# NUS-HPC-AI-Lab/VideoSys

Measured on AMD Instinct MI355X. Metric: videos/min (Open-Sora 512x512x64f, 30 denoise steps, DiT denoising only) + sec/denoise-step, higher is better.
Workload: dtype bf16; 1 GPU; open-sora-v1.2 STDiT3-XL/2 512x512x64f, latent [4,19,64,64], CFG batch 2 = 38912 token rows, 300 text tokens, depth 28; steps_per_video=30, parallelism=dsp1

## Files before the change

videosys_amd/csrc/gemm2_bf16.hip:

```cpp
#include "common.h"
#include "vsys_internal.h"

namespace vsys {
namespace {

constexpr int BM = 256, BK = 32;
constexpr int A_SLOT = BM * BK * 2;
constexpr int W_BASE = 3 * A_SLOT;
constexpr int OUT_ROW_BYTES = 96 * 2 + 16;
constexpr int OUT_WAVE_BYTES = 64 * OUT_ROW_BYTES;

template <int NWN>
struct G2 {
  static constexpr int NW = 2 * NWN;
  static constexpr int NT = 64 * NW;
  static constexpr int BN = 96 * NWN;
  static constexpr int NA = 16 / NW;
  static constexpr int W_SLOT = BN * BK * 2;
  static constexpr int WLEAD = NWN == 4 ? 2 : 1;
  static constexpr int NWSLOT = WLEAD + 1;
  static constexpr int STAGING = W_BASE + NWSLOT * W_SLOT;
  static constexpr int LDS_BYTES = STAGING > NW * OUT_WAVE_BYTES ? STAGING : NW * OUT_WAVE_BYTES;
  static constexpr int LN_BYTES = (BM + BN) * 8;
  static constexpr int KW_BYTES = 160;
};

template <int EPI, int NWN, int STAMP = 0, int MF = 0>
__global__ __launch_bounds__(G2<NWN>::NT, 2) void gemm2_kernel(GemmParams p) {
  using G = G2<NWN>;
  constexpr int BN = G::BN, NA = G::NA, W_SLOT = G::W_SLOT, WLEAD = G::WLEAD;
#if __HIP_DEVICE_COMPILE__
  extern __shared__ __attribute__((aligned(16))) char smem[];
  const int tid = threadIdx.x, lane = tid & 63, wave = tid >> 6;
  const int wm = wave / NWN, wn = wave % NWN;
  const int l31 = lane & 31, hi = lane >> 5;
  const int l15 = lane & 15, lq = lane >> 4;
  static_assert(!MF || (EPI != EPI_F32_SLICES && !STAMP), "the 16x16x32 form covers the token-row epilogues only");
  static_assert(EPI != EPI_LN_QKV_KV || (MF && NWN == 2), "the K/V epilogue exists on the 256 x 192 tile of the 16x16x32 form only");
  const int wave_u = __builtin_amdgcn_readfirstlane(wave);
  const int nbn = p.N / BN;
  int tile = xcd_remap(blockIdx.x, gridDim.x);
  int kslice = 0;
  if constexpr (EPI == EPI_F32_SLICES) {
    const int ntile = ((p.M + BM - 1) / BM) * nbn;
    kslice = tile / ntile;
    tile -= kslice * ntile;
  }
  int bm, bn;
  gemm_raster(tile, (p.M + BM - 1) / BM, nbn, p.raster_gw, p.raster_ph, bm, bn);
  const int row0 = bm * BM, col0 = bn * BN;

  const int dchunk = ((lane & 3) ^ (MF ? ((0x78 >> (2 * ((lane >> 4) & 3))) & 3) : ((lane >> 4) & 3))) * 16;
  int a_off[NA], b_off[3];
#pragma unroll
  for (int i = 0; i < NA; ++i) {
    const int r = wave_u * (16 * NA) + i * 16 + (lane >> 2);
    const int rl = row0 + r < p.M ? r : p.M - 1 - row0;
    a_off[i] = rl * (int)p.lda * 2 + dchunk;
  }
#pragma unroll
  for (int i = 0; i < 3; ++i) b_off[i] = (wave_u * 48 + i * 16 + (lane >> 2)) * (int)p.ldw * 2 + dchunk;
  const int64_t a_bytes = ((int64_t)(p.M - 1 - row0) * p.lda + p.K) * 2, b_bytes = ((int64_t)(p.N - 1 - col0) * p.ldw + p.K) * 2;
  const auto rsrc_a = __builtin_amdgcn_make_buffer_rsrc((void*)(p.A + (int64_t)row0 * p.lda), 0,
                                                        (int)(a_bytes < 0x7fffffff ? a_bytes : 0x7fffffff), 0x00020000);
  const auto rsrc_b = __builtin_amdgcn_make_buffer_rsrc((void*)(p.W + (int64_t)col0 * p.ldw), 0,
                                                        (int)(b_bytes < 0x7fffffff ? b_bytes : 0x7fffffff), 0x00020000);
  typedef __attribute__((address_space(3))) void* lds_ptr_t;
  const int kbase2 = EPI == EPI_F32_SLICES ? kslice * p.ks * 2 : 0;
  auto dma_a = [&](int i, int t, int slot) {
    __builtin_amdgcn_raw_ptr_buffer_load_lds(rsrc_a, (lds_ptr_t)(smem + slot * A_SLOT + (wave_u * (16 * NA) + i * 16) * 64), 16, a_off[i],
                                             kbase2 + t * (BK * 2), 0, 0);
  };
  auto dma_w = [&](int i, int t, int slot) {
    __builtin_amdgcn_raw_ptr_buffer_load_lds(rsrc_b, (lds_ptr_t)(smem + W_BASE + slot * W_SLOT + (wave_u * 48 + i * 16) * 64), 16,
                                             b_off[i], kbase2 + t * (BK * 2), 0, 0);
  };

  const int fsw = MF ? ((lq ^ ((0x78 >> (2 * ((l15 >> 2) & 3))) & 3)) << 4) : ((hi ^ ((l31 >> 2) & 3)) << 4);
  const int frow = MF ? l15 : l31;
  const int xo = (wm * 128 + frow) * 64 + fsw;
  const int wo = W_BASE + (wn * 96 + frow) * 64 + fsw;

  f32x16 acc[MF ? 1 : 4][MF ? 1 : 3];
  f32x4 acc16[MF ? 8 : 1][MF ? 6 : 1];
#pragma unroll
  for (int i = 0; i < (MF ? 1 : 4); ++i)
#pragma unroll
    for (int j = 0; j < (MF ? 1 : 3); ++j)
#pragma unroll
      for (int r = 0; r < 16; ++r) acc[i][j][r] = 0.f;
// ... 181 lines not shown
    }
    __builtin_amdgcn_s_barrier();
    __builtin_amdgcn_sched_barrier(0);
    if constexpr (STAMP) {
      const uint64_t now = __builtin_amdgcn_s_memtime();
      st_bar += now - st_t0; st_t0 = now;
      __builtin_amdgcn_sched_barrier(0);
    }
    sa = sa1;
    sw = sw1;
  }

  if constexpr (EPI == EPI_F32_SLICES) {
    float* o32 = p.out32 + (int64_t)kslice * p.slab;
    const int ncol0 = col0 + wn * 96;
#pragma unroll
    for (int i = 0; i < 4; ++i) {
      const int n = row0 + wm * 128 + i * 32 + l31;
      if (n < p.M) {
#pragma unroll
        for (int j = 0; j < 3; ++j)
#pragma unroll
          for (int g = 0; g < 4; ++g)
#pragma unroll
            for (int r = 0; r < 4; ++r) {
              const int m = ncol0 + j * 32 + 8 * g + 4 * hi + r;
              if (m < p.rows_per_sample) o32[(int64_t)m * p.ldo32 + n] = acc[i][j][4 * g + r];
            }
      }
    }
    return;
  }
  char* st = smem + wave * OUT_WAVE_BYTES;
  const int ncol0 = col0 + wn * 96;
  uint2 bb[3][4];
#pragma unroll
  for (int j = 0; j < 3; ++j)
#pragma unroll
    for (int g = 0; g < 4; ++g) bb[j][g] = make_uint2(0, 0);
  if (p.bias != nullptr && !LN && !MF) {
#pragma unroll
    for (int j = 0; j < 3; ++j)
#pragma unroll
      for (int g = 0; g < 4; ++g) bb[j][g] = *reinterpret_cast<const uint2*>(p.bias + ncol0 + j * 32 + 8 * g + 4 * hi);
  }
  uint2 bb16[6];
#pragma unroll
  for (int j = 0; j < 6; ++j) bb16[j] = make_uint2(0, 0);
  if (MF && p.bias != nullptr && !LN) {
#pragma unroll
    for (int j = 0; j < 6; ++j) bb16[j] = *reinterpret_cast<const uint2*>(p.bias + ncol0 + j * 16 + 4 * lq);
  }
  const bool full = row0 + BM <= p.M;
#pragma unroll
  for (int ih = 0; ih < 2; ++ih) {
    const int wrow0 = row0 + wm * 128 + ih * 64;
    if constexpr (MF) {
      if constexpr (LN) {
        float mu[4], rs[4];
#pragma unroll
        for (int i2 = 0; i2 < 4; ++i2) {
          const float2 ms = ln_lds[wm * 128 + ih * 64 + i2 * 16 + l15];
          mu[i2] = ms.x;
          rs[i2] = ms.y;
        }
#pragma unroll
        for (int j = 0; j < 6; ++j) {
          const float4* cp = reinterpret_cast<const float4*>(ln_lds + BM + wn * 96 + j * 16 + 4 * lq);
          const float4 a = cp[0], b = cp[1];
          const float c_s[4] = {a.x, a.z, b.x, b.z}, c_v[4] = {a.y, a.w, b.y, b.w};
#pragma unroll
          for (int i2 = 0; i2 < 4; ++i2) {
            const int i = ih * 4 + i2;
            const float nmu = -mu[i2], r_ = rs[i2];
            float v[4];
#pragma unroll
            for (int r = 0; r < 4; ++r) v[r] = fmaf(r_, fmaf(nmu, c_s[r], acc16[i][j][r]), c_v[r]);
            if (EPI == EPI_LN_GELU) {
#pragma unroll
              for (int r = 0; r < 4; ++r) v[r] = gelu_tanh(v[r]);
            }
            uint2 o;
            o.x = pack2bf(v[0], v[1]);
            o.y = pack2bf(v[2], v[3]);
            *reinterpret_cast<uint2*>(st + (i2 * 16 + l15) * OUT_ROW_BYTES + (j * 16 + 4 * lq) * 2) = o;
          }
        }
      } else {
        constexpr bool GATED16 = EPI == EPI_GATE_RES || EPI == EPI_GATE_RES_STATS;
        if (GATED16 && p.res != nullptr) {
#pragma unroll
          for (int half = 0; half < 2; ++half) {
            uint4 r6[6];
#pragma unroll
            for (int k = 0; k < 6; ++k) {
              const int q = lane + 64 * (6 * half + k);
              const int m_local = q / 12, c = q - m_local * 12;
              int grow = wrow0 + m_local;
              grow = grow < p.M ? grow : p.M - 1;
              r6[k] = *reinterpret_cast<const uint4*>(p.res + (int64_t)grow * p.ldr + ncol0 + c * 8);
            }
#pragma unroll
            for (int k = 0; k < 6; ++k) {
              const int q = lane + 64 * (6 * half + k);
              const int m_local = q / 12, c = q - m_local * 12;
              *reinterpret_cast<uint4*>(st + m_local * OUT_ROW_BYTES + c * 16) = r6[k];
            }
          }
          asm volatile("s_waitcnt lgkmcnt(0)" ::: "memory");
          __builtin_amdgcn_wave_barrier();
        }
#pragma unroll
        for (int i2 = 0; i2 < 4; ++i2) {
          const int i = ih * 4 + i2;
          const int m_local = i2 * 16 + l15;
          const bf16_t* gate_row = nullptr;
          if (GATED16 && p.gate != nullptr) {
            int grow = wrow0 + m_local;
            grow = grow < p.M ? grow : p.M - 1;
            const int sample = grow / p.rows_per_sample;
            gate_row = p.gate + (int64_t)sample * p.gate_stride + ncol0 + 4 * lq;
            if (p.seg_split > 0 && grow - sample * p.rows_per_sample < p.seg_split) gate_row += p.gate_alt;
          }
#pragma unroll
          for (int j = 0; j < 6; ++j) {
            uint2 gg = make_uint2(0x3f803f80u, 0x3f803f80u);
            if (GATED16 && gate_row != nullptr) gg = *reinterpret_cast<const uint2*>(gate_row + j * 16);
            float v[4];
#pragma unroll
            for (int r = 0; r < 4; ++r) v[r] = acc16[i][j][r];
            v[0] += bflo(bb16[j].x); v[1] += bfhi(bb16[j].x); v[2] += bflo(bb16[j].y); v[3] += bfhi(bb16[j].y);
            if (EPI == EPI_BIAS_GELU) {
#pragma unroll
              for (int r = 0; r < 4; ++r) v[r] = gelu_tanh(v[r]);
            }
            if (GATED16) {
              v[0] *= bflo(gg.x); v[1] *= bfhi(gg.x); v[2] *= bflo(gg.y); v[3] *= bfhi(gg.y);
            }
            uint2 o;
            o.x = pack2bf(v[0], v[1]);
            o.y = pack2bf(v[2], v[3]);
            if (GATED16 && p.res != nullptr) {
              const uint2 rr = *reinterpret_cast<const uint2*>(st + m_local * OUT_ROW_BYTES + (j * 16 + 4 * lq) * 2);
              o.x = pack2bf(bflo(o.x) + bflo(rr.x), bfhi(o.x) + bfhi(rr.x));
              o.y = pack2bf(bflo(o.y) + bflo(rr.y), bfhi(o.y) + bfhi(rr.y));
            }
            *reinterpret_cast<uint2*>(st + m_local * OUT_ROW_BYTES + (j * 16 + 4 * lq) * 2) = o;
          }
        }
        if constexpr (EPI == EPI_GATE_RES_STATS) {
          asm volatile("s_waitcnt lgkmcnt(0)" ::: "memory");
          __builtin_amdgcn_wave_barrier();
#pragma unroll
          for (int i2 = 0; i2 < 2; ++i2) {
            const int m_local = i2 * 32 + l31;
            LnAcc lacc;
#pragma unroll
            for (int j = 0; j < 3; ++j)
#pragma unroll
              for (int g = 0; g < 4; ++g) {
                const uint2 o = *reinterpret_cast<const uint2*>(st + m_local * OUT_ROW_BYTES + (j * 32 + 8 * g + 4 * hi) * 2);
                if (j == 0 && g == 0) lacc.init(bflo(o.x));
                lacc.add(bflo(o.x)); lacc.add(bfhi(o.x)); lacc.add(bflo(o.y)); lacc.add(bfhi(o.y));
              }
            const float2 mine = lacc.finish(48.f);
            const float2 other = make_float2(__shfl_xor(mine.x, 32, 64), __shfl_xor(mine.y, 32, 64));
            const float2 blk = ln_merge_equal(mine, other, 48.f);
            const int grow = wrow0 + m_local;
            if (hi == 0 && grow < p.M) p.stats_out[(int64_t)(ncol0 / LN_BLOCK) * p.stats_ld + grow] = blk;
          }
        }
      }
    } else {
    if constexpr (LN) {
      float mu[2], rs[2];
#pragma unroll
      for (int i2 = 0; i2 < 2; ++i2) {
        const float2 ms = ln_lds[wm * 128 + ih * 64 + i2 * 32 + l31];
        mu[i2] = ms.x;
        rs[i2] = ms.y;
      }
#pragma unroll
      for (int j = 0; j < 3; ++j) {
        float4 c_s[4], c_v[4];
#pragma unroll
        for (int g = 0; g < 4; ++g) {
          const float4* cp = reinterpret_cast<const float4*>(ln_lds + BM + wn * 96 + j * 32 + 8 * g + 4 * hi);
          const float4 a = cp[0], b = cp[1];
          c_s[g] = make_float4(a.x, a.z, b.x, b.z);
          c_v[g] = make_float4(a.y, a.w, b.y, b.w);
        }
#pragma unroll
        for (int i2 = 0; i2 < 2; ++i2) {
          const int i = ih * 2 + i2;
          const int m_local = i2 * 32 + l31;
          const float nmu = -mu[i2], r_ = rs[i2];
#pragma unroll
          for (int g = 0; g < 4; ++g) {
            const int n_local = j * 32 + 8 * g + 4 * hi;
            float v[4];
            v[0] = fmaf(r_, fmaf(nmu, c_s[g].x, acc[i][j][4 * g + 0]), c_v[g].x);
// ... 121 lines not shown
              const int m_local = q / 9, c = q - m_local * 9;
              kq[it] = *reinterpret_cast<const uint4*>(st + m_local * OUT_ROW_BYTES + c * 16);
            }
#pragma unroll
            for (int it = 0; it < 9; ++it) *reinterpret_cast<uint4*>(kdst + (lane + 64 * it) * 8) = kq[it];
          }
          const bool kwin = win < nq + H;
          bf16_t* vdst = p.vt + (int64_t)bt * H * 96 * p.kv_S + key0;
#pragma unroll
          for (int g = 0; g < 3; ++g) {
            uint4 o[4];
            int64_t off[4];
#pragma unroll
            for (int k = 0; k < 4; ++k) {
              const int it = g * 4 + k;
              if (kwin && it >= 3) continue;
              int col, c;
              if (kwin) {
                const int q = lane + 64 * it;
                c = q / 24;
                col = q - c * 24;
              } else {
                col = (it >> 2) * 32 + (lane & 31);
                c = 2 * (it & 3) + (lane >> 5);
              }
              const int f = vf0 + col, hv = f / 72, d = f - hv * 72;
              off[k] = ((int64_t)hv * 96 + d) * p.kv_S + c * 8;
              const char* src = st + (c * 8) * OUT_ROW_BYTES + ((kwin ? 72 : 0) + col) * 2;
              uint32_t w[4];
#pragma unroll
              for (int e = 0; e < 4; ++e)
                w[e] = (uint32_t)*reinterpret_cast<const uint16_t*>(src + (2 * e) * OUT_ROW_BYTES) |
                       ((uint32_t)*reinterpret_cast<const uint16_t*>(src + (2 * e + 1) * OUT_ROW_BYTES) << 16);
              o[k] = make_uint4(w[0], w[1], w[2], w[3]);
            }
#pragma unroll
            for (int k = 0; k < 4; ++k)
              if (!(kwin && g * 4 + k >= 3)) *reinterpret_cast<uint4*>(vdst + off[k]) = o[k];
            if (kwin) break;
          }
        }
        asm volatile("s_waitcnt lgkmcnt(0)" ::: "memory");
        __builtin_amdgcn_wave_barrier();
        continue;
      }
    }
    uint4 val[12];
#pragma unroll
    for (int it = 0; it < 12; ++it) {
      const int q = lane + 64 * it;
      const int m_local = q / 12, c = q - m_local * 12;
      val[it] = *reinterpret_cast<const uint4*>(st + m_local * OUT_ROW_BYTES + c * 16);
    }
#pragma unroll
    for (int it = 0; it < 12; ++it) {
      const int q = lane + 64 * it;
      const int m_local = q / 12, c = q - m_local * 12;
      const int64_t grow = wrow0 + m_local;
      const int gcol = ncol0 + c * 8;
      const bool ok = full || grow < p.M;
      uint4 v = val[it];
      if (EPI == EPI_GATE_RES && !MF) {
        if (p.aux != nullptr && ok) *reinterpret_cast<uint4*>(p.aux + grow * p.ldaux + gcol) = v;
        if (p.res != nullptr) {
          float a[8], b[8];
          unpack8(v, a);
          unpack8(rres[it], b);
#pragma unroll
          for (int e = 0; e < 8; ++e) a[e] += b[e];
          v = pack8(a);
        }
      }
      if (ok) *reinterpret_cast<uint4*>(p.out + grow * p.ldo + gcol) = v;
    }
    asm volatile("s_waitcnt lgkmcnt(0)" ::: "memory");
    __builtin_amdgcn_wave_barrier();
  }
  if constexpr (STAMP) {
    if (lane == 0 && p.aux != nullptr) {
      int64_t* d = reinterpret_cast<int64_t*>(p.aux) + ((int64_t)blockIdx.x * G::NW + wave) * 8;
      const uint64_t end = __builtin_amdgcn_s_memtime();
      d[0] = (int64_t)st_read; d[1] = (int64_t)st_mfma; d[2] = (int64_t)st_wait; d[3] = (int64_t)st_bar;
      d[4] = (int64_t)(st_t0 - st_begin); d[5] = (int64_t)(end - st_t0); d[6] = (int64_t)st_begin; d[7] = nt;
    }
  }
#endif
}

}

template <int NWN, int MF = 0>
static int launch_gemm2_t(const GemmParams& p, int epi, hipStream_t stream) {
  using G = G2<NWN>;
  if (p.N % G::BN != 0) return VSYS_ERR_SHAPE;
  const int nbm = (p.M + BM - 1) / BM, nbn = p.N / G::BN;
  const int grid = nbm * nbn;
  static std::atomic<unsigned long long> attr_seen{0};
  for (DeviceOnce once(attr_seen); once.todo(); once.done()) {
    (void)hipFuncSetAttribute((const void*)gemm2_kernel<EPI_BIAS, NWN, 0, MF>, hipFuncAttributeMaxDynamicSharedMemorySize, G::LDS_BYTES);
    (void)hipFuncSetAttribute((const void*)gemm2_kernel<EPI_BIAS_GELU, NWN, 0, MF>, hipFuncAttributeMaxDynamicSharedMemorySize, G::LDS_BYTES);
    (void)hipFuncSetAttribute((const void*)gemm2_kernel<EPI_GATE_RES, NWN, 0, MF>, hipFuncAttributeMaxDynamicSharedMemorySize, G::LDS_BYTES);
    (void)hipFuncSetAttribute((const void*)gemm2_kernel<EPI_LN_BIAS, NWN, 0, MF>, hipFuncAttributeMaxDynamicSharedMemorySize, G::LDS_BYTES + G::LN_BYTES);
    (void)hipFuncSetAttribute((const void*)gemm2_kernel<EPI_LN_GELU, NWN, 0, MF>, hipFuncAttributeMaxDynamicSharedMemorySize, G::LDS_BYTES + G::LN_BYTES);
    if constexpr (MF)
      (void)hipFuncSetAttribute((const void*)gemm2_kernel<EPI_GATE_RES_STATS, NWN, 0, MF>, hipFuncAttributeMaxDynamicSharedMemorySize, G::LDS_BYTES);
  }
  switch (epi) {
    case EPI_LN_BIAS: hipLaunchKernelGGL((gemm2_kernel<EPI_LN_BIAS, NWN, 0, MF>), dim3(grid), dim3(G::NT), G::LDS_BYTES + G::LN_BYTES, stream, p); break;
    case EPI_LN_GELU: hipLaunchKernelGGL((gemm2_kernel<EPI_LN_GELU, NWN, 0, MF>), dim3(grid), dim3(G::NT), G::LDS_BYTES + G::LN_BYTES, stream, p); break;
    case EPI_BIAS: hipLaunchKernelGGL((gemm2_kernel<EPI_BIAS, NWN, 0, MF>), dim3(grid), dim3(G::NT), G::LDS_BYTES, stream, p); break;
    case EPI_BIAS_GELU: hipLaunchKernelGGL((gemm2_kernel<EPI_BIAS_GELU, NWN, 0, MF>), dim3(grid), dim3(G::NT), G::LDS_BYTES, stream, p); break;
    case EPI_GATE_RES:
      if (MF && (p.aux || p.add1 || p.add2 || p.stats_out)) return VSYS_ERR_ARG;
      hipLaunchKernelGGL((gemm2_kernel<EPI_GATE_RES, NWN, 0, MF>), dim3(grid), dim3(G::NT), G::LDS_BYTES, stream, p); break;
    case EPI_GATE_RES_STATS:
      if constexpr (MF) {
        hipLaunchKernelGGL((gemm2_kernel<EPI_GATE_RES_STATS, NWN, 0, MF>), dim3(grid), dim3(G::NT), G::LDS_BYTES, stream, p);
        break;
      }
      return VSYS_ERR_ARG;
    default: return VSYS_ERR_ARG;
  }
  return hipGetLastError() == hipSuccess ? 0 : VSYS_ERR_LAUNCH;
}

int launch_gemm2_qkv_kv(const GemmParams& p_, hipStream_t stream) {
  using G = G2<2>;
  if (p_.M <= 0) return 0;
  GemmParams p = p_;
  const int H = p.kv_heads;
  if (H <= 0 || H % 8 != 0 || p.N != 216 * H || p.kv_S <= 0 || p.kv_S % 64 != 0 || p.M % p.kv_S != 0 || p.K <= 0 || p.K % BK != 0)
    return VSYS_ERR_SHAPE;
  if (!p.cs || !p.cv || !p.ln_stats || p.ln_nb < 1 || p.ln_nb > 12 || p.ln_nb * LN_BLOCK != p.K || p.ln_ld < p.M) return VSYS_ERR_SHAPE;
  if (!p.out || !p.kp || !p.vt || !p.k_norm_w || p.ldo < 72 * H) return VSYS_ERR_ARG;
  if ((p.lda % 8) || (p.ldw % 8) || (p.ldo % 8) || ((uintptr_t)p.kp % 16) || ((uintptr_t)p.vt % 16) || ((uintptr_t)p.k_norm_w % 16)) return VSYS_ERR_ALIGN;
  if (p.lda * 512 + (int64_t)p.K * 2 >= 0x7fffffff || p.ldw * 384 + (int64_t)p.K * 2 >= 0x7fffffff) return VSYS_ERR_SHAPE;
  constexpr int LDS = G::LDS_BYTES + G::LN_BYTES + G::KW_BYTES;
  static std::atomic<unsigned long long> attr_seen{0};
  for (DeviceOnce once(attr_seen); once.todo(); once.done())
    (void)hipFuncSetAttribute((const void*)gemm2_kernel<EPI_LN_QKV_KV, 2, 0, 1>, hipFuncAttributeMaxDynamicSharedMemorySize, LDS);
  const int grid = ((p.M + BM - 1) / BM) * (p.N / G::BN);
  hipLaunchKernelGGL((gemm2_kernel<EPI_LN_QKV_KV, 2, 0, 1>), dim3(grid), dim3(G::NT), LDS, stream, p);
  return hipGetLastError() == hipSuccess ? 0 : VSYS_ERR_LAUNCH;
}

#ifdef VSYS_LAB
int launch_gemm2_stamp(const GemmParams& p_, hipStream_t stream) {
  using G = G2<4>;
  GemmParams p = p_;
  p.aux = reinterpret_cast<bf16_t*>(get_lab_debug_buffer());
  if (p.N % G::BN != 0 || p.aux == nullptr) return VSYS_ERR_SHAPE;
  const int grid = ((p.M + BM - 1) / BM) * (p.N / G::BN);
  (void)hipFuncSetAttribute((const void*)gemm2_kernel<EPI_BIAS, 4, 1>, hipFuncAttributeMaxDynamicSharedMemorySize, G::LDS_BYTES);
  hipLaunchKernelGGL((gemm2_kernel<EPI_BIAS, 4, 1>), dim3(grid), dim3(G::NT), G::LDS_BYTES, stream, p);
  return hipGetLastError() == hipSuccess ? 0 : VSYS_ERR_LAUNCH;
}

#endif

int launch_gemm2_slices(const GemmParams& p, int slices, hipStream_t stream) {
  using G = G2<4>;
  if (p.M <= 0) return 0;
  if (p.N % G::BN != 0 || slices < 1 || slices > 65535 || p.ks <= 0 || p.ks % BK != 0 || p.K % BK != 0 || (int64_t)p.ks * slices < p.K ||
      (int64_t)p.ks * (slices - 1) >= p.K || p.out32 == nullptr || (p.lda % 8) || (p.ldw % 8) || p.rows_per_sample <= 0)
    return VSYS_ERR_SHAPE;
  if (p.lda * 512 + (int64_t)p.K * 2 >= 0x7fffffff || p.ldw * 768 + (int64_t)p.K * 2 >= 0x7fffffff) return VSYS_ERR_SHAPE;
  const int nbm = (p.M + BM - 1) / BM, nbn = p.N / G::BN;
  static std::atomic<unsigned long long> attr_seen{0};
  for (DeviceOnce once(attr_seen); once.todo(); once.done())
// ... 13 lines not shown
```

videosys_amd/csrc/gemm_bf16.hip:

```cpp
#include <map>
#include <mutex>

#include "common.h"
#include "vsys_internal.h"

namespace vsys {

namespace {

constexpr int BN = 192, BK = 64;
constexpr int B_BYTES = BN * BK * 2;
constexpr int OUT_ROW_BYTES = 96 * 2 + 16;
constexpr int OUT_WAVE_BYTES = 64 * OUT_ROW_BYTES;

template <int BM_>
struct Geo {
  static constexpr int NW = BM_ / 32;
  static constexpr int NT = NW * 64;
  static constexpr int A_BYTES = BM_ * BK * 2;
  static constexpr int STAGE = A_BYTES + B_BYTES;
  static constexpr int NA = 4;
  static constexpr int NB = BN / NW / 8;
  static_assert(NW * OUT_WAVE_BYTES <= 2 * STAGE, "epilogue image must fit in the staging buffers");
};
// ... 1022 lines not shown
  }
  return hipGetLastError() == hipSuccess ? 0 : VSYS_ERR_LAUNCH;
}

static bool mf16_default() {
  static const bool on = [] { const char* e = getenv("VSYS_GEMM_MF16"); return !(e && e[0] == '0'); }();
  return on;
}

namespace {
struct SplitKWs { float* ws = nullptr; int* flags = nullptr; int tiles = 0; };
std::mutex g_splitk_mutex;
std::map<hipStream_t, SplitKWs> g_splitk_ws;
}
static bool splitk_workspace(hipStream_t stream, int tiles, GemmParams& p) {
  std::lock_guard<std::mutex> lock(g_splitk_mutex);
  SplitKWs& w = g_splitk_ws[stream];
  if (w.ws == nullptr) {
    const int cap = cu_count_this_device();
    hipStreamCaptureStatus cs = hipStreamCaptureStatusNone;
    if (hipStreamIsCapturing(stream, &cs) == hipSuccess && cs != hipStreamCaptureStatusNone) return false;
    if (hipMalloc(&w.ws, (size_t)cap * 4 * 24 * 64 * sizeof(float4)) != hipSuccess) { w.ws = nullptr; return false; }
    if (hipMalloc(&w.flags, (size_t)cap * 4 * sizeof(int)) != hipSuccess || hipMemset(w.flags, 0, (size_t)cap * 4 * sizeof(int)) != hipSuccess) {
      (void)hipFree(w.ws);
      w.ws = nullptr;
      return false;
    }
    (void)hipDeviceSynchronize();
    w.tiles = cap;
  }
  if (tiles > w.tiles) return false;
  p.sk_ws = w.ws;
  p.sk_flags = w.flags;
  return true;
}
static int launch_rows128(const GemmParams& p_, int epi, hipStream_t stream, bool force_split = false) {
  if (!mf16_default() && !force_split) return launch_gemm_t<3, 128>(p_, epi, stream);
  static const bool splitk_on = [] { const char* e = getenv("VSYS_GEMM_SPLITK"); return e && e[0] == '1'; }();
  const int tiles = ((p_.M + 127) / 128) * (p_.N / BN);
  if ((splitk_on || force_split) && tiles >= 64 && tiles <= cu_count_this_device() && p_.K / BK >= 8) {
    GemmParams p = p_;
    if (splitk_workspace(stream, tiles, p)) return launch_gemm_t<3, 128, 1, 0, 1, 1>(p, epi, stream);
  }
  static const bool s8_on = [] { const char* e = getenv("VSYS_GEMM_ROWS128_S8"); return e && e[0] == '1'; }();
  if (s8_on && tiles <= cu_count_this_device() && p_.K / BK >= 3) return launch_gemm_t<8, 128, 1, 0, 1>(p_, epi, stream);
  static const bool ring_off = [] { const char* e = getenv("VSYS_GEMM_ROWS128_RING"); return e && e[0] == '0'; }();
  if (!ring_off && tiles <= cu_count_this_device() && p_.K / BK >= 3) return launch_gemm_t<9, 128, 1, 0, 1>(p_, epi, stream);
  return launch_gemm_t<3, 128, 1, 0, 1>(p_, epi, stream);
}
static int launch_sched8(const GemmParams& p, int epi, hipStream_t stream) {
  return mf16_default() ? launch_gemm_t<8, 256, 1, 0, 1>(p, epi, stream) : launch_gemm_t<8, 256>(p, epi, stream);
}

static bool ln_on_two_workgroup_tile(int64_t M, int64_t N, int64_t K) {
  return (int64_t)((M + 255) / 256) * (N / BN) >= 400 && K <= 1536 && N >= 2304 && g_gemm_variant_a.load(std::memory_order_relaxed) != 8;
}
bool gemm_ln_qkv_kv_dispatched(int64_t M, int64_t N, int64_t K) {
  return N > 0 && N % BN == 0 && K > 0 && K % BK == 0 && ln_on_two_workgroup_tile(M, N, K) && mf16_default();
}
int launch_gemm_qkv_kv(const GemmParams& p_, hipStream_t stream) {
  GemmParams p = p_;
  const int ras = g_gemm_raster_a.load(std::memory_order_relaxed);
  p.raster_gw = ras / 100;
  p.raster_ph = ras % 100;
  return launch_gemm2_qkv_kv(p, stream);
}

int launch_gemm(const GemmParams& p_, int epi, hipStream_t stream) {
  if (p_.M <= 0) return 0;
  GemmParams p = p_;
  {
    const int ras = g_gemm_raster_a.load(std::memory_order_relaxed);
    p.raster_gw = ras / 100;
    p.raster_ph = ras % 100;
  }
  if (p.N % BN != 0 || p.K % BK != 0 || p.N <= 0 || p.K <= 0) return VSYS_ERR_SHAPE;
  if ((p.lda % 8) || (p.ldw % 8) || (p.ldo % 8) || (p.res && (p.ldr % 8)) || (p.aux && (p.ldaux % 8))) return VSYS_ERR_ALIGN;
  if (p.lda * 512 + (int64_t)p.K * 2 >= 0x7fffffff || p.ldw * 384 + (int64_t)p.K * 2 >= 0x7fffffff) return VSYS_ERR_SHAPE;
  if ((epi == EPI_GATE_RES || epi == EPI_GATE_RES_STATS) && p.gate && p.rows_per_sample <= 0) return VSYS_ERR_SHAPE;
  const bool ln = epi == EPI_LN_BIAS || epi == EPI_LN_GELU;
  if (ln && (!p.cs || !p.cv || !p.ln_stats || p.ln_nb < 1 || p.ln_nb > 12 || p.ln_nb * LN_BLOCK != p.K || p.ln_ld < p.M)) return VSYS_ERR_SHAPE;
  if (epi == EPI_GATE_RES_STATS && (!p.stats_out || p.stats_ld < p.M || p.aux)) return VSYS_ERR_ARG;
  if (epi != EPI_GATE_RES && (p.add1 || p.add2)) return VSYS_ERR_ARG;
  if (epi == EPI_GATE_RES && (p.add1 || p.add2 || p.stats_out)) {
    if ((p.add2 && !p.add1) || ((p.add1 || p.add2) && (!p.res || (p.ldr % 8))) || (p.stats_out && p.stats_ld < p.M)) return VSYS_ERR_ARG;
    if ((int64_t)((p.M + 255) / 256) * (p.N / BN) < 400) return launch_rows128(p, epi, stream, g_gemm_variant_a.load(std::memory_order_relaxed) == 123);
    return g_gemm_variant_a.load(std::memory_order_relaxed) == 8 ? launch_gemm_t<8, 256>(p, epi, stream) : launch_sched8(p, epi, stream);
  }
  if (epi == EPI_GATE_RES_STATS) {
    if ((int64_t)((p.M + 255) / 256) * (p.N / BN) < 400) return launch_rows128(p, epi, stream, g_gemm_variant_a.load(std::memory_order_relaxed) == 123);
    if (g_gemm_variant_a.load(std::memory_order_relaxed) == 24) return launch_gemm2(p, epi, 2, stream);
    return g_gemm_variant_a.load(std::memory_order_relaxed) == 8 ? launch_gemm_t<8, 256>(p, epi, stream) : launch_sched8(p, epi, stream);
  }
  if (ln) {
    if ((int64_t)((p.M + 255) / 256) * (p.N / BN) < 400) return launch_rows128(p, epi, stream, g_gemm_variant_a.load(std::memory_order_relaxed) == 123);
    if (ln_on_two_workgroup_tile(p.M, p.N, p.K)) return launch_gemm2(p, epi, mf16_default() ? 2 : 0, stream);
    return g_gemm_variant_a.load(std::memory_order_relaxed) == 8 ? launch_gemm_t<8, 256>(p, epi, stream) : launch_sched8(p, epi, stream);
  }
  const int g_gemm_variant = g_gemm_variant_a.load(std::memory_order_relaxed);
  switch (g_gemm_variant == 50 ? 0 : g_gemm_variant) {
    case 6: return launch_gemm_t<6, 256>(p, epi, stream);
#ifdef VSYS_LAB
    case 18: return launch_gemm_t<18, 256>(p, epi, stream);
    case 48: return launch_gemm_t<48, 256>(p, epi, stream);
    case 38: return launch_gemm_t<38, 256>(p, epi, stream);
    case 40: return launch_gemm3(p, epi, stream);
    case 31: return (epi == EPI_BIAS && p.N % 384 == 0) ? launch_gemm2_stamp(p, stream) : VSYS_ERR_ARG;
    case 61: case 62: case 63: case 64: return epi == EPI_BIAS ? launch_gemm4_lab(p, g_gemm_variant - 60, 0, stream) : VSYS_ERR_ARG;
    case 71: case 72: case 73: case 74: case 78: return epi == EPI_BIAS ? launch_gemm4_lab(p, g_gemm_variant - 70, 1, stream) : VSYS_ERR_ARG;
    case 60: case 70: case 80:
      if (!gemm4_supports(p, epi)) return launch_gemm_t<8, 256>(p, epi, stream);
      return launch_gemm4(p, epi, (g_gemm_variant - 60) / 10, stream);
    case 81: case 82: case 83: case 84:
      return gemm4_supports(p, epi) ? launch_gemm4(p, epi, 2 + g_gemm_variant - 80, stream) : VSYS_ERR_ARG;
#endif
    case 103: return launch_gemm_t<3, 128>(p, epi, stream);
    case 113: return launch_gemm_t<3, 128, 1, 0, 1>(p, epi, stream);
    case 118: return launch_gemm_t<8, 128, 1, 0, 1>(p, epi, stream);
    case 119: return launch_gemm_t<9, 128, 1, 0, 1>(p, epi, stream);
    case 123: return launch_rows128(p, epi, stream, true);
    case 106: return launch_gemm_t<6, 128>(p, epi, stream);
    case 20: return launch_gemm2(p, epi, 0, stream);
    case 24:
      if (epi == EPI_GATE_RES && p.aux) return launch_sched8(p, epi, stream);
      return launch_gemm2(p, epi, 2, stream);
    case 30: return p.N % 384 == 0 ? launch_gemm2(p, epi, 1, stream) : launch_gemm_t<8, 256>(p, epi, stream);
    case 34: return (p.N % 384 == 0 && !(epi == EPI_GATE_RES && p.aux)) ? launch_gemm2(p, epi, 3, stream) : launch_sched8(p, epi, stream);
    case 8: return launch_gemm_t<8, 256>(p, epi, stream);
    case 16: return launch_gemm_t<8, 256, 1, 0, 1>(p, epi, stream);
    case 28: return launch_gemm_t<8, 256, 1, 1>(p, epi, stream);
    case 3: return launch_gemm_t<3, 256>(p, epi, stream);
    case 9: return launch_gemm_t<8, 256, 0>(p, epi, stream);
    default:
      if ((int64_t)((p.M + 255) / 256) * (p.N / BN) < 400) return launch_rows128(p, epi, stream, g_gemm_variant_a.load(std::memory_order_relaxed) == 123);
      if (epi != EPI_GATE_RES && p.K <= 1536 && mf16_default()) return launch_gemm2(p, epi, 2, stream);
      if (epi != EPI_GATE_RES && p.K <= 1536 && p.N >= 2304) return launch_gemm2(p, epi, 0, stream);
      if (g_gemm_variant == 50 && p.K >= 2304 && p.N % 384 == 0) return launch_gemm2(p, epi, 1, stream);
      return launch_sched8(p, epi, stream);
  }
}

int launch_linear_small(const bf16_t* x, int64_t ldx, const bf16_t* w, int64_t ldw, const bf16_t* bias, bf16_t* out,
                        int64_t ldo, int M, int N, int K, int act_in, int act_out, hipStream_t stream) {
  if (M <= 0 || N <= 0) return 0;
  if (K % 8 != 0 || (ldx % 8) || (ldw % 8)) return VSYS_ERR_ALIGN;
  const int64_t total = (int64_t)M * N;
  const int64_t grid = (total + 3) / 4;
  if (grid > 0x7fffffff) return VSYS_ERR_SHAPE;
  hipLaunchKernelGGL(linear_small_kernel, dim3((unsigned)grid), dim3(256), 0, stream, x, ldx, w, ldw, bias, out, ldo, M, N,
                     K, act_in, act_out);
  return hipGetLastError() == hipSuccess ? 0 : VSYS_ERR_LAUNCH;
}

}
```

videosys_amd/csrc/vsys_internal.h:

```cpp
#pragma once
#include <hip/hip_runtime.h>
#include <stdint.h>

#include <atomic>
#include <vector>

#include "../../include/videosys_amd.h"

namespace vsys {

typedef uint16_t bf16_t;

class DeviceOnce {
 public:
  explicit DeviceOnce(std::atomic<unsigned long long>& seen) : seen_(seen) {
    int dev = 0;
    if (hipGetDevice(&dev) == hipSuccess && dev >= 0 && dev <= 63) bit_ = 1ull << dev;
    todo_ = bit_ == 0 || (seen_.load(std::memory_order_acquire) & bit_) == 0;
  }
  bool todo() const { return todo_; }
  void done() {
    if (bit_ != 0) seen_.fetch_or(bit_, std::memory_order_release);
    todo_ = false;
  }
// ... 2 lines not shown
  std::atomic<unsigned long long>& seen_;
  unsigned long long bit_ = 0;
  bool todo_ = false;
};
inline int cu_count_this_device() {
  static std::atomic<int> cache[64];
  int dev = 0;
  if (hipGetDevice(&dev) != hipSuccess || dev < 0 || dev > 63) return 256;
  int n = cache[dev].load(std::memory_order_relaxed);
  if (n == 0) {
    hipDeviceProp_t prop;
    n = (hipGetDeviceProperties(&prop, dev) == hipSuccess && prop.multiProcessorCount > 0) ? prop.multiProcessorCount : 256;
    cache[dev].store(n, std::memory_order_relaxed);
  }
  return n;
}

enum { EPI_BIAS = VSYS_EPI_BIAS, EPI_BIAS_GELU = VSYS_EPI_BIAS_GELU, EPI_GATE_RES = VSYS_EPI_GATE_RES,
       EPI_LN_BIAS = 3, EPI_LN_GELU = 4,
       EPI_GATE_RES_STATS = 5,
       EPI_LN_QKV_KV = 6,
       EPI_F32_SLICES = 100  };
constexpr int LN_BLOCK = 96;
enum { ACT_NONE = VSYS_ACT_NONE, ACT_SILU = VSYS_ACT_SILU, ACT_GELU_TANH = VSYS_ACT_GELU_TANH };

struct GemmParams {
  const bf16_t* A; int64_t lda;
  const bf16_t* W; int64_t ldw;
  const bf16_t* bias;
  bf16_t* out; int64_t ldo;
  int M, N, K;
  const bf16_t* gate; int64_t gate_stride;
  const bf16_t* res; int64_t ldr;
  bf16_t* aux; int64_t ldaux;
  int rows_per_sample;
  int seg_split; int64_t gate_alt;
  int ks; float* out32; int64_t slab, ldo32;
  const float* cs = nullptr; const float* cv = nullptr;
  const float2* ln_stats = nullptr; int64_t ln_ld = 0; int ln_nb = 0; float ln_eps = 0.f;
  float2* stats_out = nullptr; int64_t stats_ld = 0;
  const bf16_t* add1 = nullptr; const bf16_t* add2 = nullptr;
  int raster_gw = 6, raster_ph = 0;
  float* sk_ws = nullptr; int* sk_flags = nullptr;
  bf16_t* kp = nullptr; bf16_t* vt = nullptr; const bf16_t* k_norm_w = nullptr;
  int kv_S = 0, kv_heads = 0; float k_eps = 0.f, kscale = 0.f;
};

__host__ __device__ inline int qkv_kv_column(int n, int heads) {
  const int C = 72 * heads, nq = C / 96;
  if (n < C) return n;
  if (n < 2 * C) return (nq + (n - C) / 72) * 96 + (n - C) % 72;
  const int f = n - 2 * C;
  return f < 24 * heads ? (nq + f / 24) * 96 + 72 + f % 24 : (nq + heads) * 96 + (f - 24 * heads);
}

struct ConvParams {
  const bf16_t* A; int64_t lda;
  const bf16_t* W; int64_t ldw;
  const bf16_t* bias;
  const bf16_t* res; int64_t ldr;
  bf16_t* out; float* out32; int64_t ldo;
  int M, N, K;
  int cin, taps, cshift, taps_hw, kw, row_pitch, plane_pitch, max_tap_rows;
  int batch; int64_t batch_a, batch_w, batch_o;
  float out_scale;
};
int launch_conv(const ConvParams& p, hipStream_t stream);

struct VaeGrid {
  int T, H, W, pad, tf;
  int64_t sample_rows;
};
int launch_gn_stats(const bf16_t* x, const VaeGrid& g, int N, int C, int groups, float eps, float* partial, int nblk, float* stats,
                    hipStream_t stream);
int launch_gn_apply(const bf16_t* x, const VaeGrid& gs, bf16_t* y, const VaeGrid& gd, int N, int C, int groups, const float* stats,
                    const bf16_t* gamma, const bf16_t* beta, int act, hipStream_t stream);
int launch_regrid(const bf16_t* x, const VaeGrid& gs, bf16_t* y, const VaeGrid& gd, int N, int C, int up, int tmode, hipStream_t stream);
int launch_subsample(const bf16_t* x, const VaeGrid& gs, bf16_t* y, const VaeGrid& gd, int N, int C, int st, int ss, int t0, int s0,
                     hipStream_t stream);
int launch_spatial_norm_apply(const bf16_t* x, const VaeGrid& gs, bf16_t* y, const VaeGrid& gd, int N, int C, int groups,
                              const float* stats, const bf16_t* gamma, const bf16_t* beta, const bf16_t* yb, int zT, int zH, int zW,
                              hipStream_t stream);
int launch_blend_edge(const bf16_t* a, bf16_t* b, int64_t outer, int Ha, int Wa, int Hb, int Wb, int ext, int axis, hipStream_t stream);
int launch_d2s_time(const bf16_t* x, const VaeGrid& gs, bf16_t* y, const VaeGrid& gd, int N, int Cout, hipStream_t stream);
int launch_vae_first_im2col(const bf16_t* z, int F, int H, int W, int kt, int kcols, const float* scale, const float* shift,
                            const float* pq_w, const float* pq_b, bf16_t* out, hipStream_t stream);
int launch_extract_planar(const bf16_t* x, const VaeGrid& g, int N, int ldx, int nc, int tskip, bf16_t* out, int64_t Ftot, int f0,
                          hipStream_t stream);
int launch_softmax_rows(const float* s, bf16_t* p, int64_t rows, int n, int ld, hipStream_t stream);

int launch_gather_rows(const bf16_t* table, const int64_t* ids, bf16_t* out, int64_t n, int C, int64_t vocab, hipStream_t stream);
int launch_rms_norm_rows(const bf16_t* x, const bf16_t* w, bf16_t* y, int64_t rows, int C, float eps, hipStream_t stream);
int launch_geglu(const bf16_t* h, bf16_t* out, int64_t rows, int F, hipStream_t stream);
int launch_t5_attention(const bf16_t* qkv, int64_t row_stride, int inner, const float* relbias, const int* klen, bf16_t* out,
                        int64_t out_stride, int B, int L, int heads, hipStream_t stream);
int launch_splitk_reduce_t(const float* part, int S, int64_t slab, int ldp, const bf16_t* res, int64_t ldr, bf16_t* out, int64_t ldo,
                           int M, int N, hipStream_t stream);
int launch_splitk_reduce(const float* part, int S, int64_t slab, int64_t ldp, const bf16_t* res, int64_t ldr, bf16_t* out, int64_t ldo,
                         int M, int N, hipStream_t stream);
int launch_t5_attention_mfma(const bf16_t* qkv, int64_t row_stride, int inner, const float* bias, int bias_ld, int bias_center,
                             int kv_len, bf16_t* kp, bf16_t* vt, bf16_t* out, int64_t out_stride, int L, int heads,
                             hipStream_t stream);

int launch_gemm(const GemmParams& p, int epi, hipStream_t stream);
int launch_gemm2(const GemmParams& p, int epi, int wide, hipStream_t stream);
int launch_gemm2_qkv_kv(const GemmParams& p, hipStream_t stream);
// ... 99 lines not shown
```

videosys_amd/ops.py:

```python
from __future__ import annotations

from typing import Optional

import torch

from . import _lib, program

EPI_BIAS, EPI_BIAS_GELU, EPI_GATE_RES = 0, 1, 2
ACT_NONE, ACT_SILU, ACT_GELU_TANH = 0, 1, 2
HEAD_DIM = 72
VT_ROWS = 96


class _TPtr(int):
    """A device address that remembers its tensor: ctypes and the launch-program recorder see the integer, the custom-op route
    (torch.ops.vsys.launch) hands the TENSOR to the dispatcher."""


def _p(t: Optional[torch.Tensor]):
    if t is None:
        return None
    if program.active() is not None:
        program.keep(t)
    a = _TPtr(t.data_ptr())
# ... 297 lines not shown

def copy_4d(src, dst, n0, n1, n2, C, sstr, dstr, n1_valid=None, n2_valid=None):
    _chk(src, dst)
    _bf16(src, dst)
    lib = _lib.load()
    _call("vsys_copy_4d", _p(src), _p(dst), n0, n1, n2, C, sstr[0], sstr[1], sstr[2], dstr[0], dstr[1], dstr[2],
                                n1 if n1_valid is None else n1_valid, n2 if n2_valid is None else n2_valid)
    return dst


def copy_4d_batch(src, dst, descs):
    import ctypes

    _chk(src, dst)
    _bf16(src, dst)
    lib = _lib.load()
    for i in range(0, len(descs), 16):
        part = descs[i:i + 16]
        flat = [int(v) for d in part for v in d]
        arr = (ctypes.c_int64 * len(flat))(*flat)
        _call("vsys_copy_4d_batch", _p(src), _p(dst), len(part), arr)


def kv_pad_len(kv_len: int) -> int:
    return (kv_len + 63) // 64 * 64


def alloc_kv_buffers(batch, heads, kv_len, device):
    kv_pad = kv_pad_len(kv_len)
    kp = torch.zeros(batch, heads, kv_pad, HEAD_DIM, dtype=torch.bfloat16, device=device)
    vt = torch.zeros(batch, heads, VT_ROWS, kv_pad, dtype=torch.bfloat16, device=device)
    return kp, vt


def _fused_kv_default() -> bool:
    import os

    return os.environ.get("VSYS_FUSED_KV", "1") != "0"


FUSED_KV = _fused_kv_default()


def qkv_kv_column_order(heads: int) -> torch.Tensor:
    assert heads > 0 and heads % 4 == 0
    C, nq = 72 * heads, 72 * heads // 96
    n = torch.arange(3 * C, dtype=torch.int64)
    k, f = n - C, n - 2 * C
    kcol = (nq + k // 72) * 96 + k % 72
    vcol = torch.where(f < 24 * heads, (nq + f // 24) * 96 + 72 + f % 24, (nq + heads) * 96 + (f - 24 * heads))
    return torch.where(n < C, n, torch.where(n < 2 * C, kcol, vcol))


def gemm_ln_qkv_kv_dispatched(M: int, N: int, K: int) -> bool:
    return bool(_lib.load().vsys_gemm_bf16_ln_qkv_kv_dispatched(M, N, K))


def kv_set_constant_rows(vt):
    assert vt.shape[2] == VT_ROWS
    vt[:, :, HEAD_DIM:] = 0
    vt[:, :, HEAD_DIM] = 1.0
    vt[:, :, HEAD_DIM + 4] = 1.0


def gemm_ln_qkv_kv(x, wp, cs, cv, stats, k_norm_w, q, kp, vt, S, heads, eps=1e-6, k_eps=1e-6):
    _chk(x, wp, cs, cv, stats, k_norm_w, q, kp, vt)
    _bf16(x, wp, k_norm_w, q, kp, vt)
    assert x.dim() == 2 and x.stride(1) == 1 and wp.stride(1) == 1 and q.stride(1) == 1 and cs.dtype == torch.float32 and cv.dtype == torch.float32
    M, K = x.shape
    assert wp.shape == (216 * heads, K) and cs.numel() == cv.numel() == 216 * heads and k_norm_w.numel() == HEAD_DIM and k_norm_w.is_contiguous()
    assert S > 0 and M % S == 0 and q.shape[0] == M and q.shape[1] >= HEAD_DIM * heads and kp.is_contiguous() and vt.is_contiguous()
    assert tuple(kp.shape) == (M // S, heads, S, HEAD_DIM) and tuple(vt.shape) == (M // S, heads, VT_ROWS, S)
    ld = _stats_ld(stats, M, K // LN_BLOCK)
    _call("vsys_gemm_bf16_ln_qkv_kv", _p(x), x.stride(0), _p(wp), wp.stride(0), _p(cs), _p(cv), _p(stats), ld, _p(k_norm_w), _p(q),
          q.stride(0), _p(kp), _p(vt), M, K, S, heads, float(eps), float(k_eps))
    return q


def attn_prep_kv(k, v, k_norm_w, kp, vt, batch, heads, kv_len, eps=1e-6):
    _chk(k, v, k_norm_w, kp, vt)
    _bf16(k, v, k_norm_w, kp, vt)
    assert k.stride(1) == 1 and v.stride(1) == 1 and kp.is_contiguous() and vt.is_contiguous()
    kv_pad = kp.shape[2]
    assert vt.shape[3] == kv_pad and vt.shape[2] == VT_ROWS
    lib = _lib.load()
    _call("vsys_attn_prep_kv", _p(k), k.stride(0), _p(v), v.stride(0), _p(k_norm_w), _p(kp), _p(vt), batch, heads,
                                     kv_len, kv_pad, eps)


def flash_attn(q, q_norm_w, kp, vt, out, batch, heads, q_len, kv_len, eps=1e-6, k_norm_bound=None, keys_exact=False):
    _chk(q, q_norm_w, kp, vt, out)
    _bf16(q, q_norm_w, kp, vt, out)
    assert q.stride(1) == 1 and out.stride(1) == 1
    kv_pad = kp.shape[2]
    if keys_exact and not k_norm_bound:
        _call("vsys_flash_attn_d72_exact", _p(q), q.stride(0), _p(q_norm_w), _p(kp), _p(vt), _p(out), out.stride(0), batch, heads,
              q_len, kv_len, kv_pad, eps)
    elif k_norm_bound:
        _call("vsys_flash_attn_d72_kb", _p(q), q.stride(0), _p(q_norm_w), _p(kp), _p(vt), _p(out), out.stride(0), batch, heads,
              q_len, kv_len, kv_pad, eps, float(k_norm_bound))
    else:
        _call("vsys_flash_attn_d72", _p(q), q.stride(0), _p(q_norm_w), _p(kp), _p(vt), _p(out), out.stride(0), batch, heads,
              q_len, kv_len, kv_pad, eps)
    return out


# ... 430 lines not shown
```

Baseline: 20.70 videos/min.

## Route gated-residual GEMMs to the two-workgroup tile with async residual DMA into LDS

```diff
diff --git a/videosys_amd/csrc/gemm2_bf16.hip b/videosys_amd/csrc/gemm2_bf16.hip
--- a/videosys_amd/csrc/gemm2_bf16.hip
+++ b/videosys_amd/csrc/gemm2_bf16.hip
@@ -36,6 +36,7 @@
   const int l31 = lane & 31, hi = lane >> 5;
   const int l15 = lane & 15, lq = lane >> 4;
   static_assert(!MF || (EPI != EPI_F32_SLICES && !STAMP), "the 16x16x32 form covers the token-row epilogues only");
+  constexpr bool GATED16 = MF && (EPI == EPI_GATE_RES || EPI == EPI_GATE_RES_STATS);
   static_assert(EPI != EPI_LN_QKV_KV || (MF && NWN == 2), "the K/V epilogue exists on the 256 x 192 tile of the 16x16x32 form only");
   const int wave_u = __builtin_amdgcn_readfirstlane(wave);
   const int nbn = p.N / BN;
@@ -323,6 +324,28 @@
     for (int j = 0; j < 6; ++j) bb16[j] = *reinterpret_cast<const uint2*>(p.bias + ncol0 + j * 16 + 4 * lq);
   }
   const bool full = row0 + BM <= p.M;
+  const int64_t r_bytes = ((int64_t)(p.M - 1 - row0) * p.ldr + (p.N - col0)) * 2;
+  const auto rsrc_r = __builtin_amdgcn_make_buffer_rsrc((void*)(p.res + (int64_t)row0 * p.ldr + col0), 0,
+                                                        (int)(r_bytes < 0x7fffffff ? r_bytes : 0x7fffffff), 0x00020000);
+  auto res_dma = [&](int ih) {
+    int m_local, c;
+    gated_res_landing(0, lane, m_local, c);
+#pragma unroll
+    for (int it = 0; it < 13; ++it) {
+      const int r = (wave_u / NWN) * 128 + ih * 64 + m_local, rlast = p.M - 1 - row0;
+      const int rl = r < rlast ? r : rlast;
+      const int data = (c - 12) >> 31;
+      const int off = ((rl * (int)p.ldr * 2 + ((wave_u % NWN) * 96 + c * 8) * 2) & data) | (0x7ffffff0 & ~data);
+      __builtin_amdgcn_raw_ptr_buffer_load_lds(rsrc_r, (lds_ptr_t)(smem + wave_u * OUT_WAVE_BYTES + it * 1024), 16, off, 0, 0, 0);
+      __builtin_amdgcn_sched_barrier(0);
+      c += 12;
+      m_local += 4;
+      if (c >= 13) { c -= 13; m_local += 1; }
+    }
+  };
+  if constexpr (GATED16) {
+    if (p.res != nullptr) res_dma(0);
+  }
 #pragma unroll
   for (int ih = 0; ih < 2; ++ih) {
     const int wrow0 = row0 + wm * 128 + ih * 64;
@@ -358,45 +381,77 @@
           }
         }
       } else {
-        constexpr bool GATED16 = EPI == EPI_GATE_RES || EPI == EPI_GATE_RES_STATS;
-        if (GATED16 && p.res != nullptr) {
-#pragma unroll
-          for (int half = 0; half < 2; ++half) {
-            uint4 r6[6];
-#pragma unroll
-            for (int k = 0; k < 6; ++k) {
-              const int q = lane + 64 * (6 * half + k);
-              const int m_local = q / 12, c = q - m_local * 12;
-              int grow = wrow0 + m_local;
+        if constexpr (GATED16) {
+          const int wrow0_u = row0 + (wave_u / NWN) * 128 + ih * 64;
+          bool uni = true;
+          const bf16_t* gate_u = nullptr;
+          if (p.gate != nullptr) {
+            const int first = wrow0_u < p.M ? wrow0_u : p.M - 1, last = wrow0_u + 63 < p.M ? wrow0_u + 63 : p.M - 1;
+            const int s0 = first / p.rows_per_sample, s1 = last / p.rows_per_sample;
+            const bool alt0 = p.seg_split > 0 && first - s0 * p.rows_per_sample < p.seg_split;
+            const bool alt1 = p.seg_split > 0 && last - s1 * p.rows_per_sample < p.seg_split;
+            uni = s0 == s1 && alt0 == alt1;
+            gate_u = p.gate + (int64_t)s0 * p.gate_stride + (alt0 ? p.gate_alt : 0) + ncol0 + 4 * lq;
+          }
+          auto conv = [&](int i2, int j, uint2 gg) {
+            const int m_local = i2 * 16 + l15;
+            float v[4];
+#pragma unroll
+            for (int r = 0; r < 4; ++r) v[r] = acc16[ih * 4 + i2][j][r];
+            v[0] += bflo(bb16[j].x); v[1] += bfhi(bb16[j].x); v[2] += bflo(bb16[j].y); v[3] += bfhi(bb16[j].y);
+            v[0] *= bflo(gg.x); v[1] *= bfhi(gg.x); v[2] *= bflo(gg.y); v[3] *= bfhi(gg.y);
+            uint2 o;
+            o.x = pack2bf(v[0], v[1]);
+            o.y = pack2bf(v[2], v[3]);
+            uint2* cell = reinterpret_cast<uint2*>(st + m_local * OUT_ROW_BYTES + (j * 16 + 4 * lq) * 2);
+            if (p.res != nullptr) {
+              const uint2 rr = *cell;
+              o.x = pack2bf(bflo(o.x) + bflo(rr.x), bfhi(o.x) + bfhi(rr.x));
+              o.y = pack2bf(bflo(o.y) + bflo(rr.y), bfhi(o.y) + bfhi(rr.y));
+            }
+            *cell = o;
+          };
+          if (uni) {
+            uint2 gg6[6];
+#pragma unroll
+            for (int j = 0; j < 6; ++j) gg6[j] = make_uint2(0x3f803f80u, 0x3f803f80u);
+            if (gate_u != nullptr) {
+#pragma unroll
+              for (int j = 0; j < 6; ++j) gg6[j] = *reinterpret_cast<const uint2*>(gate_u + j * 16);
+            }
+            asm volatile("s_waitcnt vmcnt(0)" ::: "memory");
+            __builtin_amdgcn_wave_barrier();
+#pragma unroll
+            for (int i2 = 0; i2 < 4; ++i2)
+#pragma unroll
+              for (int j = 0; j < 6; ++j) conv(i2, j, gg6[j]);
+          } else {
+            int64_t goff[4];
+#pragma unroll
+            for (int i2 = 0; i2 < 4; ++i2) {
+              int grow = wrow0 + i2 * 16 + l15;
               grow = grow < p.M ? grow : p.M - 1;
-              r6[k] = *reinterpret_cast<const uint4*>(p.res + (int64_t)grow * p.ldr + ncol0 + c * 8);
-            }
-#pragma unroll
-            for (int k = 0; k < 6; ++k) {
-              const int q = lane + 64 * (6 * half + k);
-              const int m_local = q / 12, c = q - m_local * 12;
-              *reinterpret_cast<uint4*>(st + m_local * OUT_ROW_BYTES + c * 16) = r6[k];
-            }
-          }
-          asm volatile("s_waitcnt lgkmcnt(0)" ::: "memory");
-          __builtin_amdgcn_wave_barrier();
-        }
+              const int sample = grow / p.rows_per_sample;
+              goff[i2] = (int64_t)sample * p.gate_stride + ((p.seg_split > 0 && grow - sample * p.rows_per_sample < p.seg_split) ? p.gate_alt : 0);
+            }
+            asm volatile("s_waitcnt vmcnt(0)" ::: "memory");
+            __builtin_amdgcn_wave_barrier();
+#pragma unroll
+            for (int j = 0; j < 6; ++j) {
+              uint2 gg4[4];
+#pragma unroll
+              for (int i2 = 0; i2 < 4; ++i2) gg4[i2] = *reinterpret_cast<const uint2*>(p.gate + goff[i2] + ncol0 + 4 * lq + j * 16);
+#pragma unroll
+              for (int i2 = 0; i2 < 4; ++i2) conv(i2, j, gg4[i2]);
+            }
+          }
+        } else {
 #pragma unroll
         for (int i2 = 0; i2 < 4; ++i2) {
           const int i = ih * 4 + i2;
           const int m_local = i2 * 16 + l15;
-          const bf16_t* gate_row = nullptr;
-          if (GATED16 && p.gate != nullptr) {
-            int grow = wrow0 + m_local;
-            grow = grow < p.M ? grow : p.M - 1;
-            const int sample = grow / p.rows_per_sample;
-            gate_row = p.gate + (int64_t)sample * p.gate_stride + ncol0 + 4 * lq;
-            if (p.seg_split > 0 && grow - sample * p.rows_per_sample < p.seg_split) gate_row += p.gate_alt;
-          }
 #pragma unroll
           for (int j = 0; j < 6; ++j) {
-            uint2 gg = make_uint2(0x3f803f80u, 0x3f803f80u);
-            if (GATED16 && gate_row != nullptr) gg = *reinterpret_cast<const uint2*>(gate_row + j * 16);
             float v[4];
 #pragma unroll
             for (int r = 0; r < 4; ++r) v[r] = acc16[i][j][r];
@@ -405,19 +460,12 @@
 #pragma unroll
               for (int r = 0; r < 4; ++r) v[r] = gelu_tanh(v[r]);
             }
-            if (GATED16) {
-              v[0] *= bflo(gg.x); v[1] *= bfhi(gg.x); v[2] *= bflo(gg.y); v[3] *= bfhi(gg.y);
-            }
             uint2 o;
             o.x = pack2bf(v[0], v[1]);
             o.y = pack2bf(v[2], v[3]);
-            if (GATED16 && p.res != nullptr) {
-              const uint2 rr = *reinterpret_cast<const uint2*>(st + m_local * OUT_ROW_BYTES + (j * 16 + 4 * lq) * 2);
-              o.x = pack2bf(bflo(o.x) + bflo(rr.x), bfhi(o.x) + bfhi(rr.x));
-              o.y = pack2bf(bflo(o.y) + bflo(rr.y), bfhi(o.y) + bfhi(rr.y));
-            }
             *reinterpret_cast<uint2*>(st + m_local * OUT_ROW_BYTES + (j * 16 + 4 * lq) * 2) = o;
           }
+        }
         }
         if constexpr (EPI == EPI_GATE_RES_STATS) {
           asm volatile("s_waitcnt lgkmcnt(0)" ::: "memory");
@@ -645,6 +693,13 @@
       const int m_local = q / 12, c = q - m_local * 12;
       val[it] = *reinterpret_cast<const uint4*>(st + m_local * OUT_ROW_BYTES + c * 16);
     }
+    if constexpr (GATED16) {
+      if (ih == 0 && p.res != nullptr) {
+        asm volatile("s_waitcnt lgkmcnt(0)" ::: "memory");
+        __builtin_amdgcn_wave_barrier();
+        res_dma(1);
+      }
+    }
 #pragma unroll
     for (int it = 0; it < 12; ++it) {
       const int q = lane + 64 * it;
@@ -705,9 +760,11 @@
     case EPI_BIAS_GELU: hipLaunchKernelGGL((gemm2_kernel<EPI_BIAS_GELU, NWN, 0, MF>), dim3(grid), dim3(G::NT), G::LDS_BYTES, stream, p); break;
     case EPI_GATE_RES:
       if (MF && (p.aux || p.add1 || p.add2 || p.stats_out)) return VSYS_ERR_ARG;
+      if (MF && p.res && p.ldr * 512 + (int64_t)p.N * 2 >= 0x7fffffff) return VSYS_ERR_SHAPE;
       hipLaunchKernelGGL((gemm2_kernel<EPI_GATE_RES, NWN, 0, MF>), dim3(grid), dim3(G::NT), G::LDS_BYTES, stream, p); break;
     case EPI_GATE_RES_STATS:
       if constexpr (MF) {
+        if (p.res && p.ldr * 512 + (int64_t)p.N * 2 >= 0x7fffffff) return VSYS_ERR_SHAPE;
         hipLaunchKernelGGL((gemm2_kernel<EPI_GATE_RES_STATS, NWN, 0, MF>), dim3(grid), dim3(G::NT), G::LDS_BYTES, stream, p);
         break;
       }
diff --git a/videosys_amd/csrc/gemm_bf16.hip b/videosys_amd/csrc/gemm_bf16.hip
--- a/videosys_amd/csrc/gemm_bf16.hip
+++ b/videosys_amd/csrc/gemm_bf16.hip
@@ -1098,6 +1098,12 @@
   return mf16_default() ? launch_gemm_t<8, 256, 1, 0, 1>(p, epi, stream) : launch_gemm_t<8, 256>(p, epi, stream);
 }
 
+static bool gated_on_two_workgroup_tile(const GemmParams& p) {
+  static const bool on = [] { const char* e = getenv("VSYS_GATED_GEMM2"); return !(e && e[0] == '0'); }();
+  return on && mf16_default() && p.K <= 1536 && (int64_t)((p.M + 255) / 256) * (p.N / BN) >= 400 &&
+         !(p.res && p.ldr * 512 + (int64_t)p.N * 2 >= 0x7fffffff);
+}
+
 static bool ln_on_two_workgroup_tile(int64_t M, int64_t N, int64_t K) {
   return (int64_t)((M + 255) / 256) * (N / BN) >= 400 && K <= 1536 && N >= 2304 && g_gemm_variant_a.load(std::memory_order_relaxed) != 8;
 }
@@ -1136,6 +1142,7 @@
   if (epi == EPI_GATE_RES_STATS) {
     if ((int64_t)((p.M + 255) / 256) * (p.N / BN) < 400) return launch_rows128(p, epi, stream, g_gemm_variant_a.load(std::memory_order_relaxed) == 123);
     if (g_gemm_variant_a.load(std::memory_order_relaxed) == 24) return launch_gemm2(p, epi, 2, stream);
+    if (g_gemm_variant_a.load(std::memory_order_relaxed) == 0 && gated_on_two_workgroup_tile(p)) return launch_gemm2(p, epi, 2, stream);
     return g_gemm_variant_a.load(std::memory_order_relaxed) == 8 ? launch_gemm_t<8, 256>(p, epi, stream) : launch_sched8(p, epi, stream);
   }
   if (ln) {
@@ -1181,6 +1188,7 @@
       if ((int64_t)((p.M + 255) / 256) * (p.N / BN) < 400) return launch_rows128(p, epi, stream, g_gemm_variant_a.load(std::memory_order_relaxed) == 123);
       if (epi != EPI_GATE_RES && p.K <= 1536 && mf16_default()) return launch_gemm2(p, epi, 2, stream);
       if (epi != EPI_GATE_RES && p.K <= 1536 && p.N >= 2304) return launch_gemm2(p, epi, 0, stream);
+      if (epi == EPI_GATE_RES && !p.aux && g_gemm_variant == 0 && gated_on_two_workgroup_tile(p)) return launch_gemm2(p, epi, 2, stream);
       if (g_gemm_variant == 50 && p.K >= 2304 && p.N % 384 == 0) return launch_gemm2(p, epi, 1, stream);
       return launch_sched8(p, epi, stream);
   }
diff --git a/videosys_amd/csrc/vsys_internal.h b/videosys_amd/csrc/vsys_internal.h
--- a/videosys_amd/csrc/vsys_internal.h
+++ b/videosys_amd/csrc/vsys_internal.h
@@ -78,6 +78,12 @@
   if (n < 2 * C) return (nq + (n - C) / 72) * 96 + (n - C) % 72;
   const int f = n - 2 * C;
   return f < 24 * heads ? (nq + f / 24) * 96 + 72 + f % 24 : (nq + heads) * 96 + (f - 24 * heads);
+}
+
+__host__ __device__ inline void gated_res_landing(int piece, int lane, int& m, int& c) {
+  const int q = 64 * piece + lane;
+  m = q / 13;
+  c = q - 13 * m;
 }
 
 struct ConvParams {
diff --git a/videosys_amd/ops.py b/videosys_amd/ops.py
--- a/videosys_amd/ops.py
+++ b/videosys_amd/ops.py
@@ -373,6 +373,12 @@
     return torch.where(n < C, n, torch.where(n < 2 * C, kcol, vcol))
 
 
+def _gated_res_landing(piece: int, lane: int):
+    assert 0 <= piece < 13 and 0 <= lane < 64
+    m, c = divmod(64 * piece + lane, 13)
+    return m, (c if c < 12 else None)
+
+
 def gemm_ln_qkv_kv_dispatched(M: int, N: int, K: int) -> bool:
     return bool(_lib.load().vsys_gemm_bf16_ln_qkv_kv_dispatched(M, N, K))
 
```

After: 20.81 videos/min (median of 6 runs). About the same (+0.5%).
